# sash-a/CleanRL.jl

Measured on NVIDIA B200. Metric: ppo_env_steps_per_sec, higher is better.
Workload: dtype f32

## Files before the change

### cleanrl.jl_b200/csrc/rollout.cu

```cuda
#include "kernels.h"
#include "mlp_tile.cuh"

namespace {

constexpr int RE = 32;
constexpr int ROLL_FWD = CRL_THREADS;
constexpr int ROLL_THREADS = ROLL_FWD + 64;
constexpr int BIG_FWD = 128, BIG_THREADS = BIG_FWD + 64;
constexpr int BAR_FWD = 1, BAR_SPEC = 2, BAR_BOOK = 3;

__device__ __forceinline__ void nbar_sync(int id, int n) { asm volatile("bar.sync %0, %1;" ::"r"(id), "r"(n) : "memory"); }
__device__ __forceinline__ void nbar_arrive(int id, int n) { asm volatile("bar.arrive %0, %1;" ::"r"(id), "r"(n) : "memory"); }

template <int ENV> struct RolloutSmem {
  using G = TileGeom<4, 2>;
  using E = EnvTraits<ENV>;
  static constexpr int SP = G::S_PAD;
  static constexpr int PARAMS = 0;
  static constexpr int X = PARAMS + SmemParams<ENV>::SIZE;
  static constexpr int H1 = X + CRL_MAXD * SP;
  static constexpr int H2 = H1 + G::ROWS * SP;
  static constexpr int OUT = H2 + G::ROWS * SP;
  static constexpr int ST = OUT + 4 * RE;
  static constexpr int SPEC = ST + 4 * RE;
  static constexpr int RST = SPEC + 2 * 4 * RE;
  static constexpr int NOISE = RST + 4 * RE;
  static constexpr int USED = NOISE + 2 * RE;
  static constexpr int BOOK = USED + RE;
  static constexpr int FLOATS = BOOK + 4 * RE;
  static constexpr size_t BYTES = FLOATS * sizeof(float);
  static_assert((NOISE % 2) == 0, "the Float64 uniforms need 8-byte alignment");
};

#ifdef ROLL_TRACE
#define RTR(i) do { if (tr) tr[i] = clock64(); } while (0)
#else
#define RTR(i) do { } while (0)
#endif

template <int ENV> struct HeadRow { float w[CRL_H]; float b; };
template <int ENV> __device__ __forceinline__ void load_head_row(const float* sp, HeadRow<ENV>& hr) {
  using E = EnvTraits<ENV>;
  const int o = threadIdx.x / RE;
#pragma unroll
  for (int k = 0; k < CRL_H; k++) hr.w[k] = 0.0f;
  hr.b = 0.0f;
  if (threadIdx.x >= RE * (E::A + 1)) return;
  if (o < E::A) {
    const float* a = sp + SmemParams<ENV>::ACTOR;
#pragma unroll
    for (int k = 0; k < CRL_H; k++) hr.w[k] = a[NetOff<E::D, E::A>::W3 + k * E::A + o];
    hr.b = a[NetOff<E::D, E::A>::B3 + o];
  } else {
    const float* c = sp + SmemParams<ENV>::CRITIC;
#pragma unroll
    for (int k = 0; k < CRL_H; k++) hr.w[k] = c[NetOff<E::D, 1>::W3 + k];
    hr.b = c[NetOff<E::D, 1>::B3];
  }
}

template <int ENV, bool HEADREG = true, bool BOOKSYNC = false>
__device__ __forceinline__ void forward32(const ThreadCoord<TileGeom<4, 2>>& tc, float* smem, const HeadRow<ENV>& hr,
                                          long long* tr = nullptr) {
  using G = TileGeom<4, 2>;
  using E = EnvTraits<ENV>;
  using SM = RolloutSmem<ENV>;
  constexpr int SP = G::S_PAD;
  float* sp = smem + SM::PARAMS;
  float* xs = smem + SM::X;
  float* h1 = smem + SM::H1;
  float* h2 = smem + SM::H2;
  float* so = smem + SM::OUT;
  const float* np = sp + net_base<ENV>(tc.net);
  using NO = NetOff<E::D, 1>;
  RTR(0);
  tile_layer_fwd4<G, E::D>(tc, np + NO::W1, np + NO::B1, xs, h1 + tc.net * CRL_H * SP);
  RTR(1);
  nbar_sync(BAR_FWD, ROLL_FWD);
  RTR(2);
  tile_layer_fwd4<G, CRL_H>(tc, np + NO::W2, np + NO::B2, h1 + tc.net * CRL_H * SP, h2 + tc.net * CRL_H * SP);
  RTR(3);
  nbar_sync(BAR_FWD, ROLL_FWD);
  RTR(4);
  if (threadIdx.x < RE * (E::A + 1)) {
    const int o = threadIdx.x / RE, e = threadIdx.x % RE;
    const float* hrow = h2 + (o < E::A ? 0 : CRL_H) * SP + e;
    float hv[CRL_H];
#pragma unroll
    for (int k = 0; k < CRL_H; k++) hv[k] = hrow[k * SP];
    if (BOOKSYNC) nbar_sync(BAR_BOOK, RE * (E::A + 1) + 32);
    float acc = 0.0f;
    if (HEADREG) {
#pragma unroll
      for (int k = 0; k < CRL_H; k++) acc = fmaf(hr.w[k], hv[k], acc);
      acc += hr.b;
    } else if (o < E::A) {
      const float* a = sp + SmemParams<ENV>::ACTOR;
#pragma unroll
      for (int k = 0; k < CRL_H; k++) acc = fmaf(a[NetOff<E::D, E::A>::W3 + k * E::A + o], hv[k], acc);
      acc += a[NetOff<E::D, E::A>::B3 + o];
    } else {
      const float* c = sp + SmemParams<ENV>::CRITIC;
#pragma unroll
      for (int k = 0; k < CRL_H; k++) acc = fmaf(c[NetOff<E::D, 1>::W3 + k], hv[k], acc);
      acc += c[NetOff<E::D, 1>::B3];
    }
    so[o * RE + e] = acc;
  }
  RTR(5);
  nbar_sync(BAR_FWD, ROLL_FWD);
  RTR(6);
}

struct FwdCoord8x4 {
  int q, p, net, nb;
  __device__ FwdCoord8x4() {
    const int lane = threadIdx.x & 31, w = (threadIdx.x >> 5) & 3;
    q = w * 4 + (lane >> 3);
    p = lane & 7;
    net = q >> 3;
    nb = 8 * (q & 7);
  }
};
template <int K>
__device__ __forceinline__ void fwd_layer_8x4(const FwdCoord8x4& fc, const float* __restrict__ Wt, const float* __restrict__ bias,
                                              const float* __restrict__ in, float* __restrict__ out) {
  constexpr int SP = RE + 4, PF = 2;
  const float* wp = Wt + fc.nb;
  const float* ap = in + 4 * fc.p;
  const float4 b0 = *reinterpret_cast<const float4*>(bias + fc.nb), b1 = *reinterpret_cast<const float4*>(bias + fc.nb + 4);
  float2 acc[8][2];
#pragma unroll
  for (int j = 0; j < 8; j++) acc[j][0] = acc[j][1] = make_float2(0.0f, 0.0f);
  float4 w0[PF], w1[PF], av[PF];
#pragma unroll
  for (int i = 0; i < PF; i++) {
    if (i < K) {
      w0[i] = *reinterpret_cast<const float4*>(wp + i * CRL_H);
      w1[i] = *reinterpret_cast<const float4*>(wp + i * CRL_H + 4);
      av[i] = *reinterpret_cast<const float4*>(ap + i * SP);
    }
  }
#pragma unroll
  for (int k0 = 0; k0 < K; k0 += PF) {
    float4 w0n[PF], w1n[PF], avn[PF];
#pragma unroll
    for (int i = 0; i < PF; i++) {
      if (k0 + PF + i < K) {
        w0n[i] = *reinterpret_cast<const float4*>(wp + (k0 + PF + i) * CRL_H);
        w1n[i] = *reinterpret_cast<const float4*>(wp + (k0 + PF + i) * CRL_H + 4);
        avn[i] = *reinterpret_cast<const float4*>(ap + (k0 + PF + i) * SP);
      }
    }
#pragma unroll
    for (int i = 0; i < PF; i++) {
      if (k0 + i < K) {
        const float2 a01 = make_float2(av[i].x, av[i].y), a23 = make_float2(av[i].z, av[i].w);
#pragma unroll
        for (int j = 0; j < 8; j++) {
          const float wj = j < 4 ? f4_get(w0[i], j) : f4_get(w1[i], j - 4);
          const float2 ww = make_float2(wj, wj);
          acc[j][0] = __ffma2_rn(ww, a01, acc[j][0]);
          acc[j][1] = __ffma2_rn(ww, a23, acc[j][1]);
        }
      }
    }
#pragma unroll
    for (int i = 0; i < PF; i++) { w0[i] = w0n[i]; w1[i] = w1n[i]; av[i] = avn[i]; }
  }
#pragma unroll
  for (int j = 0; j < 8; j++) {
    const float b = j < 4 ? f4_get(b0, j) : f4_get(b1, j - 4);
    const float2 t0 = tanh_fast2(__fadd2_rn(acc[j][0], make_float2(b, b)));
    const float2 t1 = tanh_fast2(__fadd2_rn(acc[j][1], make_float2(b, b)));
    *reinterpret_cast<float4*>(out + (fc.nb + j) * SP + 4 * fc.p) = make_float4(t0.x, t0.y, t1.x, t1.y);
  }
}
template <int ENV, bool BOOKSYNC = false>
__device__ __forceinline__ void forward32_big(const FwdCoord8x4& fc, float* smem) {
  using E = EnvTraits<ENV>;
  using SM = RolloutSmem<ENV>;
  constexpr int SP = RE + 4;
  static_assert(SP == TileGeom<4, 2>::S_PAD, "both forward variants share one activation layout");
  float* sp = smem + SM::PARAMS;
  float* xs = smem + SM::X;
  float* h1 = smem + SM::H1;
  float* h2 = smem + SM::H2;
  float* so = smem + SM::OUT;
  const float* np = sp + net_base<ENV>(fc.net);
  using NO = NetOff<E::D, 1>;
  fwd_layer_8x4<E::D>(fc, np + NO::W1, np + NO::B1, xs, h1 + fc.net * CRL_H * SP);
  nbar_sync(BAR_FWD, BIG_FWD);
  fwd_layer_8x4<CRL_H>(fc, np + NO::W2, np + NO::B2, h1 + fc.net * CRL_H * SP, h2 + fc.net * CRL_H * SP);
  nbar_sync(BAR_FWD, BIG_FWD);
  if (threadIdx.x < RE * (E::A + 1)) {
    const int o = threadIdx.x / RE, e = threadIdx.x % RE;
    const float* hrow = h2 + (o < E::A ? 0 : CRL_H) * SP + e;
    if (BOOKSYNC) nbar_sync(BAR_BOOK, RE * (E::A + 1) + 32);
    float acc = 0.0f;
    if (o < E::A) {
      const float* a = sp + SmemParams<ENV>::ACTOR;
#pragma unroll 16
      for (int k = 0; k < CRL_H; k++) acc = fmaf(a[NetOff<E::D, E::A>::W3 + k * E::A + o], hrow[k * SP], acc);
      acc += a[NetOff<E::D, E::A>::B3 + o];
    } else {
      const float* c = sp + SmemParams<ENV>::CRITIC;
#pragma unroll 16
      for (int k = 0; k < CRL_H; k++) acc = fmaf(c[NetOff<E::D, 1>::W3 + k], hrow[k * SP], acc);
      acc += c[NetOff<E::D, 1>::B3];
    }
    so[o * RE + e] = acc;
  }
  nbar_sync(BAR_FWD, BIG_FWD);
}

template <int ENV, bool BIG>
__global__ void __launch_bounds__(BIG ? BIG_THREADS : ROLL_THREADS, BIG ? 2 : 1) rollout_kernel(RolloutArgs a) {
  constexpr int FWD = BIG ? BIG_FWD : ROLL_FWD;
  constexpr int SW0 = FWD / 32;
  using G = TileGeom<4, 2>;
  using E = EnvTraits<ENV>;
  using SM = RolloutSmem<ENV>;
  constexpr int SP = G::S_PAD;
  constexpr int D = E::D, A = E::A, S = E::S;
  constexpr bool CART = ENV == CRL_ENV_CARTPOLE;
  extern __shared__ __align__(16) float smem[];
  float* sp = smem + SM::PARAMS;
  float* xs = smem + SM::X;
  float* so = smem + SM::OUT;
  float* st_s = smem + SM::ST;
  float* spec_s = smem + SM::SPEC;
  float* rst_s = smem + SM::RST;
  double* noise_d = reinterpret_cast<double*>(smem + SM::NOISE);
  float* noise_f = smem + SM::NOISE;
  int* used_s = reinterpret_cast<int*>(smem + SM::USED);
  int* act_s = reinterpret_cast<int*>(smem + SM::BOOK);
  float* actf_s = smem + SM::BOOK + RE;
  float* rew_s = smem + SM::BOOK + 2 * RE;
  int* done_s = reinterpret_cast<int*>(smem + SM::BOOK + 3 * RE);
  const ThreadCoord<G> tc;
  const FwdCoord8x4 fc;

  load_params<ENV>(a.params, sp);
  for (int i = threadIdx.x; i < CRL_MAXD * SP; i += blockDim.x) xs[i] = 0.0f;

  const int warp = threadIdx.x >> 5;
  const int e = threadIdx.x & 31;
  const long long n = (long long)blockIdx.x * RE + e;
  const bool fwd = threadIdx.x < FWD;
  const bool owner = threadIdx.x < RE;
  const bool booker = warp == SW0 + 1;
  const bool in_range = n < a.N;
  const bool valid = owner && in_range;
  const unsigned long long step0 = a.ds->policy_step;
  const uint32_t gid = (uint32_t)(a.env_id_base + (int)n);

  float st[S];
  float obs[D];
  int env_t = 0;
  uint32_t resets = 0;
  bool done_flag = false;
  int ep_len = 0;
  double ep_ret = 0.0;
  bool prev_done = false;
  float obs_b[D];
  unsigned long long agg_n = 0;
  double agg_ret = 0.0, agg_len = 0.0, agg_max = -INFINITY;
  bool rec_pending = false;
  unsigned int rec_slot = 0;
  crl_episode rec;
  rec.step = 0; rec.env = 0; rec.length = 0; rec._pad = 0; rec.episode_return = 0.0;

#pragma unroll
  for (int i = 0; i < S; i++) st[i] = 0.0f;
#pragma unroll
  for (int k = 0; k < D; k++) obs_b[k] = 0.0f;
  if (valid) {
#pragma unroll
    for (int i = 0; i < S; i++) st[i] = a.env_state[n * S + i];
    env_t = a.env_t[n];
    resets = a.reset_count[n];
  }
  if (booker && in_range) {
    ep_len = a.ep_length[n];
    ep_ret = a.ep_return[n];
    resets = a.reset_count[n];
  }
  __syncthreads();
  HeadRow<ENV> hr;
  if (!BIG) load_head_row<ENV>(sp, hr);
  if (owner) {
    env_obs<ENV>(st, obs);
#pragma unroll
    for (int k = 0; k < D; k++) xs[k * SP + e] = obs[k];
#pragma unroll
    for (int i = 0; i < S; i++) st_s[i * RE + e] = st[i];
    used_s[e] = 0;
  }
  auto prepare_reset = [&]() {
    float u4[4], rs[S];
    int rt;
    rng_reset_uniforms(a.seed, gid, resets, u4);
    env_reset<ENV>(rs, rt, u4);
#pragma unroll
    for (int i = 0; i < S; i++) rst_s[i * RE + e] = rs[i];
  };
  if (booker && !a.reset_noise) prepare_reset();

  auto book = [&](int tb, const float (&zv)[A + 1], int act_i, float act_f, float r, bool dn) {
    const long long b = (long long)tb * a.N + n;
    ep_len += 1;
    float logprob;
    if (!E::CONT) {
      float m = zv[0];
#pragma unroll
      for (int k = 1; k < A; k++) m = fmaxf(m, zv[k]);
      float sum = 0.0f;
#pragma unroll
      for (int k = 0; k < A; k++) sum = __fadd_rn(sum, expf(__fsub_rn(zv[k], m)));
      const float ls = logf(sum);
      logprob = __fsub_rn(__fsub_rn(zv[0], m), ls);
#pragma unroll
      for (int k = 1; k < A; k++) logprob = (act_i == k) ? __fsub_rn(__fsub_rn(zv[k], m), ls) : logprob;
    } else {
      float lps = 0.0f;
#pragma unroll
      for (int k = 0; k < A; k++) {
        const float mean = zv[k];
        const float logstd = sp[SmemParams<ENV>::LOGSTD + k];
        const float sd = expf(logstd);
        const float diff = __fsub_rn(act_f, mean);
        const float q = __fdiv_rn(-__fmul_rn(diff, diff), __fmul_rn(__fmul_rn(2.0f, sd), sd));
        lps = __fadd_rn(lps, __fsub_rn(__fsub_rn(q, logstd), 0.9189385332046727f));
      }
      logprob = lps;
    }
    if (rec_pending) {
      if (rec_slot < (unsigned int)a.ep_capacity) a.records[rec_slot] = rec;
      rec_pending = false;
    }
    ep_ret += (double)r;
    if (in_range) {
      if (D == 4) {
        reinterpret_cast<float4*>(a.state)[b] = make_float4(obs_b[0], obs_b[1], obs_b[2], obs_b[3]);
      } else {
#pragma unroll
        for (int k = 0; k < D; k++) a.state[b * D + k] = obs_b[k];
      }
      if (!E::CONT) reinterpret_cast<int32_t*>(a.action)[b] = act_i;
      else reinterpret_cast<float*>(a.action)[b * A] = act_f;
      a.logprob[b] = logprob;
      a.value[b] = zv[A];
      a.terminal[b] = prev_done ? 1 : 0;
      a.reward[b] = r;
      if (dn) {
        rec_slot = atomicAdd(&a.eb->count, 1u);
        rec_pending = true;
        rec.step = tb; rec.env = (int)n; rec.length = ep_len; rec._pad = 0; rec.episode_return = ep_ret;
        agg_n += 1; agg_ret += ep_ret; agg_len += (double)ep_len; agg_max = fmax(agg_max, ep_ret);
        ep_ret = 0.0;
        ep_len = 0;
      }
    }
    prev_done = dn;
  };
  static_assert(!E::CONT || A == 1, "the Gaussian head hands one action per env to the bookkeeping warp");
  __syncthreads();

  for (int t = 0; t < a.T; t++) {
    if (!fwd) {
      if (booker) {
        float zv[A + 1];
#pragma unroll
        for (int k = 0; k <= A; k++) zv[k] = so[k * RE + e];
        const int act_i = act_s[e];
        const float act_f = actf_s[e], r = rew_s[e];
        const bool dn = done_s[e] != 0;
        nbar_arrive(BAR_BOOK, RE * (A + 1) + 32);
        if (t > 0) book(t - 1, zv, act_i, act_f, r, dn);
#pragma unroll
        for (int k = 0; k < D; k++) obs_b[k] = xs[k * SP + e];
        if (!a.reset_noise && used_s[e]) {
          resets += 1;
          prepare_reset();
          used_s[e] = 0;
        }
      }
      if (warp == SW0 && !a.action_noise) {
        if (!E::CONT) {
          noise_d[e] = in_range ? rng_action_uniform(a.seed, gid, step0 + (unsigned long long)t) : 0.0;
        } else {
          float zn[2] = {0.0f, 0.0f};
          if (in_range) rng_action_normals(a.seed, gid, step0 + (unsigned long long)t, zn);
          noise_f[e] = zn[0];
          noise_f[RE + e] = zn[1];
        }
      }
      if (CART) {
        float s4[4];
#pragma unroll
        for (int i = 0; i < 4; i++) s4[i] = st_s[i * RE + e];
        cartpole_dynamics(s4, warp - SW0);
#pragma unroll
        for (int i = 0; i < 4; i++) spec_s[((warp - SW0) * 4 + i) * RE + e] = s4[i];
      }
      __threadfence_block();
      nbar_arrive(BAR_SPEC, RE + 64);
    } else {
      if (BIG) forward32_big<ENV, true>(fc, smem); else forward32<ENV, true, true>(tc, smem, hr);
      if (owner) {
        const long long b = (long long)t * a.N + n;
        int act_i = 0;
        float act_f = 0.0f;
        if (!E::CONT) {
          float z[A], p[A];
#pragma unroll
          for (int k = 0; k < A; k++) z[k] = so[k * RE + e];
          float m = z[0];
#pragma unroll
          for (int k = 1; k < A; k++) m = fmaxf(m, z[k]);
          float ex[A], sum = 0.0f;
#pragma unroll
          for (int k = 0; k < A; k++) { ex[k] = expf(__fsub_rn(z[k], m)); sum = __fadd_rn(sum, ex[k]); }
          float psum = 0.0f;
#pragma unroll
          for (int k = 0; k < A; k++) {
            p[k] = __fdiv_rn(ex[k], sum);
            psum = __fadd_rn(psum, p[k]);
          }
          nbar_sync(BAR_SPEC, RE + 64);
          double u = 0.0;
          if (valid) u = a.action_noise ? a.action_noise[b] : noise_d[e];
          const double tt = __dmul_rn(u, (double)psum);
          float cw = p[0];
          int i = 0;
#pragma unroll
          for (int k = 1; k < A; k++) {
            if ((double)cw < tt && i == k - 1) { i = k; cw = __fadd_rn(cw, p[k]); }
          }
          act_i = i;
        } else {
          nbar_sync(BAR_SPEC, RE + 64);
          float zn = 0.0f;
          if (valid) zn = a.action_noise ? (float)a.action_noise[b * A] : noise_f[e];
          const float mean = so[e];
          const float sd = expf(sp[SmemParams<ENV>::LOGSTD]);
          act_f = __fadd_rn(mean, __fmul_rn(sd, zn));
        }
        float r;
        bool dn;
        if (CART) {
#pragma unroll
          for (int i = 0; i < 4; i++) st[i] = spec_s[(act_i * 4 + i) * RE + e];
          env_t += 1;
          cartpole_outcome(st, env_t, a.max_steps, r, dn);
        } else {
          pendulum_step(st, env_t, act_f, a.max_steps, r, dn);
        }
        env_obs<ENV>(st, obs);
        done_flag = dn;
        act_s[e] = act_i; actf_s[e] = act_f; rew_s[e] = r; done_s[e] = dn ? 1 : 0;
        if (valid && dn) {
          if (a.reset_noise) {
            const float4 v = reinterpret_cast<const float4*>(a.reset_noise)[b];
            const float u4[4] = {v.x, v.y, v.z, v.w};
            env_reset<ENV>(st, env_t, u4);
          } else {
#pragma unroll
            for (int i = 0; i < S; i++) st[i] = rst_s[i * RE + e];
            env_t = 0;
            used_s[e] = 1;
          }
          resets += 1;
          if (a.fresh_obs_after_reset) env_obs<ENV>(st, obs);
        }
#pragma unroll
        for (int k = 0; k < D; k++) xs[k * SP + e] = obs[k];
#pragma unroll
        for (int i = 0; i < S; i++) st_s[i * RE + e] = st[i];
      }
    }
    __syncthreads();
  }
  if (!fwd) {
    if (booker) {
      float zv[A + 1];
#pragma unroll
      for (int k = 0; k <= A; k++) zv[k] = so[k * RE + e];
      const int act_i = act_s[e];
      const float act_f = actf_s[e], r = rew_s[e];
      const bool dn = done_s[e] != 0;
      nbar_arrive(BAR_BOOK, RE * (A + 1) + 32);
      book(a.T - 1, zv, act_i, act_f, r, dn);
      if (rec_pending && rec_slot < (unsigned int)a.ep_capacity) a.records[rec_slot] = rec;
      if (in_range) {
        a.ep_length[n] = ep_len;
        a.ep_return[n] = ep_ret;
      }
      const double sr = warp_sum(agg_ret), sl = warp_sum(agg_len), mx = warp_max(agg_max);
      unsigned long long cn = agg_n;
#pragma unroll
      for (int o = 16; o > 0; o >>= 1) cn += __shfl_xor_sync(0xffffffffu, cn, o);
      if (e == 0 && cn > 0) {
        atomicAdd(&a.eb->n_episodes, cn);
        atomicAdd(&a.eb->sum_return, sr);
        atomicAdd(&a.eb->sum_length, sl);
        unsigned long long* addr = reinterpret_cast<unsigned long long*>(&a.eb->max_return);
        unsigned long long old = *addr, assumed;
        do {
          assumed = old;
          if (__longlong_as_double((long long)assumed) >= mx) break;
          old = atomicCAS(addr, assumed, (unsigned long long)__double_as_longlong(mx));
        } while (assumed != old);
      }
    }
    return;
  }

  float obs_last[D];
#pragma unroll
  for (int k = 0; k < D; k++) obs_last[k] = obs[k];
  if (owner) {
    float fresh[D];
    env_obs<ENV>(st, fresh);
#pragma unroll
    for (int k = 0; k < D; k++) xs[k * SP + e] = fresh[k];
  }
  nbar_sync(BAR_FWD, FWD);
  if (BIG) forward32_big<ENV, true>(fc, smem); else forward32<ENV, true, true>(tc, smem, hr);
  if (valid) {
    a.next_value[n] = so[A * RE + e];
#pragma unroll
    for (int i = 0; i < S; i++) a.env_state[n * S + i] = st[i];
    a.env_t[n] = env_t;
    a.reset_count[n] = resets;
#pragma unroll
    for (int k = 0; k < D; k++) a.next_obs[n * D + k] = obs_last[k];
    a.next_done[n] = done_flag ? 1 : 0;
  }
}

template <int ENV>
__global__ void env_step_raw_kernel(float* state, int* t, const void* action, float* reward, uint8_t* done,
                                    long long n, int max_steps) {
  constexpr int S = EnvTraits<ENV>::S;
  const long long i = (long long)blockIdx.x * blockDim.x + threadIdx.x;
  if (i >= n) return;
  float st[S];
#pragma unroll
  for (int k = 0; k < S; k++) st[k] = state[i * S + k];
  int tt = t[i];
  float r;
  bool dn;
  if (ENV == CRL_ENV_CARTPOLE) cartpole_step(st, tt, reinterpret_cast<const int32_t*>(action)[i], max_steps, r, dn);
  else pendulum_step(st, tt, reinterpret_cast<const float*>(action)[i], max_steps, r, dn);
#pragma unroll
  for (int k = 0; k < S; k++) state[i * S + k] = st[k];
  t[i] = tt;
  reward[i] = r;
  done[i] = dn ? 1 : 0;
}

template <int ENV>
__global__ void __launch_bounds__(CRL_THREADS) policy_forward_raw_kernel(const float* params, const float* obs,
                                                                         float* out_policy, float* logp,
                                                                         float* value, long long n) {
  using G = TileGeom<4, 2>;
  using E = EnvTraits<ENV>;
  using SM = RolloutSmem<ENV>;
  constexpr int SP = G::S_PAD;
  constexpr int D = E::D, A = E::A;
  extern __shared__ __align__(16) float smem[];
  float* xs = smem + SM::X;
  float* so = smem + SM::OUT;
  const ThreadCoord<G> tc;
  load_params<ENV>(params, smem + SM::PARAMS);
  const int e = threadIdx.x;
  const long long i = (long long)blockIdx.x * RE + e;
  if (e < RE) {
#pragma unroll
    for (int k = 0; k < D; k++) xs[k * SP + e] = i < n ? obs[i * D + k] : 0.0f;
  }
  __syncthreads();
  HeadRow<ENV> hr;
  load_head_row<ENV>(smem + SM::PARAMS, hr);
  forward32<ENV>(tc, smem, hr);
  if (e < RE && i < n) {
    float z[A];
#pragma unroll
    for (int k = 0; k < A; k++) { z[k] = so[k * RE + e]; out_policy[i * A + k] = z[k]; }
    value[i] = so[A * RE + e];
    if (!E::CONT) {
      float m = z[0];
#pragma unroll
      for (int k = 1; k < A; k++) m = fmaxf(m, z[k]);
      float sum = 0.0f;
#pragma unroll
      for (int k = 0; k < A; k++) sum = __fadd_rn(sum, expf(__fsub_rn(z[k], m)));
      const float ls = logf(sum);
#pragma unroll
      for (int k = 0; k < A; k++) logp[i * A + k] = __fsub_rn(__fsub_rn(z[k], m), ls);
    }
  }
}

template <int ENV> cudaError_t launch_rollout_t(const RolloutArgs& a, cudaStream_t s) {
  const int grid = (a.N + RE - 1) / RE;
  static int sms = 0;
  if (sms == 0) {
    int dev = 0;
    cudaGetDevice(&dev);
    cudaDeviceGetAttribute(&sms, cudaDevAttrMultiProcessorCount, dev);
  }
  if (grid > sms) rollout_kernel<ENV, true><<<grid, BIG_THREADS, RolloutSmem<ENV>::BYTES, s>>>(a);
  else rollout_kernel<ENV, false><<<grid, ROLL_THREADS, RolloutSmem<ENV>::BYTES, s>>>(a);
  return cudaGetLastError();
}

template <int ENV>
cudaError_t launch_policy_forward_t(const float* params, const float* obs, float* out_policy, float* logp,
                                    float* value, long long n, cudaStream_t s) {
  const long long grid = (n + RE - 1) / RE;
  if (grid == 0) return cudaSuccess;
  policy_forward_raw_kernel<ENV><<<(unsigned)grid, CRL_THREADS, RolloutSmem<ENV>::BYTES, s>>>(params, obs, out_policy,
                                                                                              logp, value, n);
  return cudaGetLastError();
}

__global__ void episode_buf_init_kernel(EpisodeBuf* eb) {
  eb->count = 0; eb->_pad = 0; eb->n_episodes = 0ull; eb->sum_return = 0.0; eb->sum_length = 0.0;
  eb->max_return = -INFINITY;
}

template <int ENV> cudaError_t init_attrs_t() {
  cudaError_t e = cudaFuncSetAttribute(rollout_kernel<ENV, false>, cudaFuncAttributeMaxDynamicSharedMemorySize,
                                       (int)RolloutSmem<ENV>::BYTES);
  if (e != cudaSuccess) return e;
  e = cudaFuncSetAttribute(rollout_kernel<ENV, true>, cudaFuncAttributeMaxDynamicSharedMemorySize, (int)RolloutSmem<ENV>::BYTES);
  if (e != cudaSuccess) return e;
  return cudaFuncSetAttribute(policy_forward_raw_kernel<ENV>, cudaFuncAttributeMaxDynamicSharedMemorySize,
                              (int)RolloutSmem<ENV>::BYTES);
}

}

cudaError_t kernels_init_rollout() {
  cudaError_t e = init_attrs_t<CRL_ENV_CARTPOLE>();
  if (e != cudaSuccess) return e;
  return init_attrs_t<CRL_ENV_PENDULUM>();
}

cudaError_t launch_episode_buf_init(EpisodeBuf* eb, cudaStream_t s) {
  episode_buf_init_kernel<<<1, 1, 0, s>>>(eb);
  return cudaGetLastError();
}

cudaError_t launch_rollout(int env_kind, const RolloutArgs& a, cudaStream_t s) {
  return env_kind == CRL_ENV_CARTPOLE ? launch_rollout_t<CRL_ENV_CARTPOLE>(a, s) : launch_rollout_t<CRL_ENV_PENDULUM>(a, s);
}

cudaError_t launch_env_step_raw(int env_kind, float* state, int* t, const void* action, float* reward,
                                uint8_t* done, long long n, int max_steps, cudaStream_t s) {
  if (n == 0) return cudaSuccess;
  const unsigned grid = (unsigned)((n + 127) / 128);
  if (env_kind == CRL_ENV_CARTPOLE)
    env_step_raw_kernel<CRL_ENV_CARTPOLE><<<grid, 128, 0, s>>>(state, t, action, reward, done, n, max_steps);
  else
    env_step_raw_kernel<CRL_ENV_PENDULUM><<<grid, 128, 0, s>>>(state, t, action, reward, done, n, max_steps);
  return cudaGetLastError();
}

cudaError_t launch_policy_forward_raw(int env_kind, const float* params, const float* obs, float* out_policy,
                                      float* logp, float* value, long long n, cudaStream_t s) {
  return env_kind == CRL_ENV_CARTPOLE
             ? launch_policy_forward_t<CRL_ENV_CARTPOLE>(params, obs, out_policy, logp, value, n, s)
             : launch_policy_forward_t<CRL_ENV_PENDULUM>(params, obs, out_policy, logp, value, n, s);
}

namespace {
template <int ENV>
__global__ void env_reset_kernel(int N, unsigned long long seed, int env_id_base, float* env_state, int* env_t,
                                 double* ep_return, int* ep_length, uint32_t* reset_count, float* next_obs,
                                 uint8_t* next_done) {
  constexpr int S = EnvTraits<ENV>::S, D = EnvTraits<ENV>::D;
  const int n = blockIdx.x * blockDim.x + threadIdx.x;
  if (n >= N) return;
  float u4[4], st[S], obs[D];
  const uint32_t k = reset_count[n];
  rng_reset_uniforms(seed, (uint32_t)(env_id_base + n), k, u4);
  int t;
  env_reset<ENV>(st, t, u4);
  env_obs<ENV>(st, obs);
#pragma unroll
  for (int i = 0; i < S; i++) env_state[n * S + i] = st[i];
#pragma unroll
  for (int i = 0; i < D; i++) next_obs[n * D + i] = obs[i];
  env_t[n] = t;
  reset_count[n] = k + 1;
  next_done[n] = 0;
  ep_return[n] = 0.0;
  ep_length[n] = 0;
}
template <int ENV>
__global__ void env_refresh_kernel(int N, const float* env_state, float* next_obs, uint8_t* next_done) {
  constexpr int S = EnvTraits<ENV>::S, D = EnvTraits<ENV>::D;
  const int n = blockIdx.x * blockDim.x + threadIdx.x;
  if (n >= N) return;
  float st[S], obs[D];
#pragma unroll
  for (int i = 0; i < S; i++) st[i] = env_state[n * S + i];
  env_obs<ENV>(st, obs);
#pragma unroll
  for (int i = 0; i < D; i++) next_obs[n * D + i] = obs[i];
  next_done[n] = 0;
}
}

cudaError_t launch_env_reset(int env_kind, int N, unsigned long long seed, int env_id_base, float* env_state,
                             int* env_t, double* ep_return, int* ep_length, uint32_t* reset_count, float* next_obs,
                             uint8_t* next_done, cudaStream_t s) {
  const int grid = (N + 127) / 128;
  if (env_kind == CRL_ENV_CARTPOLE)
    env_reset_kernel<CRL_ENV_CARTPOLE><<<grid, 128, 0, s>>>(N, seed, env_id_base, env_state, env_t, ep_return, ep_length,
                                                           reset_count, next_obs, next_done);
  else
    env_reset_kernel<CRL_ENV_PENDULUM><<<grid, 128, 0, s>>>(N, seed, env_id_base, env_state, env_t, ep_return, ep_length,
                                                           reset_count, next_obs, next_done);
  return cudaGetLastError();
}

cudaError_t launch_env_refresh(int env_kind, int N, const float* env_state, float* next_obs, uint8_t* next_done,
                               cudaStream_t s) {
  const int grid = (N + 127) / 128;
  if (env_kind == CRL_ENV_CARTPOLE) env_refresh_kernel<CRL_ENV_CARTPOLE><<<grid, 128, 0, s>>>(N, env_state, next_obs, next_done);
  else env_refresh_kernel<CRL_ENV_PENDULUM><<<grid, 128, 0, s>>>(N, env_state, next_obs, next_done);
  return cudaGetLastError();
}
```

Measured before the change: 249.9 million.

## Precompute first-layer activations for both CartPole action candidates speculatively

While the forward warps finish the current step, idle forward warps now compute layer-1 hidden activations for both speculative next CartPole states (one per discrete action). The next step's layer 1 is then a select between the two precomputed candidates, keyed on the chosen action stored in smem. This takes layer 1 off the serial critical path at the cost of doubling layer-1 work, adding another named barrier and using more shared memory. It only applies to the small-grid CartPole path without fresh observations after reset.

```diff
diff --git a/cleanrl.jl_b200/csrc/rollout.cu b/cleanrl.jl_b200/csrc/rollout.cu
--- a/cleanrl.jl_b200/csrc/rollout.cu
+++ b/cleanrl.jl_b200/csrc/rollout.cu
@@ -8,6 +8,8 @@
 constexpr int ROLL_THREADS = ROLL_FWD + 64;
 constexpr int BIG_FWD = 128, BIG_THREADS = BIG_FWD + 64;
 constexpr int BAR_FWD = 1, BAR_SPEC = 2, BAR_BOOK = 3;
+constexpr int BAR_CAND = 4;
+constexpr int CAND_THREADS = 192;
 
 __device__ __forceinline__ void nbar_sync(int id, int n) { asm volatile("bar.sync %0, %1;" ::"r"(id), "r"(n) : "memory"); }
 __device__ __forceinline__ void nbar_arrive(int id, int n) { asm volatile("bar.arrive %0, %1;" ::"r"(id), "r"(n) : "memory"); }
@@ -29,6 +31,9 @@
   static constexpr int BOOK = USED + RE;
   static constexpr int FLOATS = BOOK + 4 * RE;
   static constexpr size_t BYTES = FLOATS * sizeof(float);
+  static constexpr int XC = FLOATS;
+  static constexpr int HC = XC + 2 * CRL_MAXD * SP;
+  static constexpr size_t CAND_BYTES = (HC + 2 * G::ROWS * SP) * sizeof(float);
   static_assert((NOISE % 2) == 0, "the Float64 uniforms need 8-byte alignment");
 };
 
@@ -61,7 +66,7 @@
 
 template <int ENV, bool HEADREG = true, bool BOOKSYNC = false>
 __device__ __forceinline__ void forward32(const ThreadCoord<TileGeom<4, 2>>& tc, float* smem, const HeadRow<ENV>& hr,
-                                          long long* tr = nullptr) {
+                                          bool l1_cand = false, long long* tr = nullptr) {
   using G = TileGeom<4, 2>;
   using E = EnvTraits<ENV>;
   using SM = RolloutSmem<ENV>;
@@ -74,7 +79,20 @@
   const float* np = sp + net_base<ENV>(tc.net);
   using NO = NetOff<E::D, 1>;
   RTR(0);
-  tile_layer_fwd4<G, E::D>(tc, np + NO::W1, np + NO::B1, xs, h1 + tc.net * CRL_H * SP);
+  if (l1_cand) {
+    const float* hc = smem + SM::HC;
+    const int4 act = *reinterpret_cast<const int4*>(smem + SM::BOOK + tc.sb[0]);
+#pragma unroll
+    for (int j = 0; j < 4; j++) {
+      const int off = (tc.net * CRL_H + tc.jb[0] + j) * SP + tc.sb[0];
+      const float4 c0 = *reinterpret_cast<const float4*>(hc + off);
+      const float4 c1 = *reinterpret_cast<const float4*>(hc + G::ROWS * SP + off);
+      *reinterpret_cast<float4*>(h1 + off) =
+          make_float4(act.x ? c1.x : c0.x, act.y ? c1.y : c0.y, act.z ? c1.z : c0.z, act.w ? c1.w : c0.w);
+    }
+  } else {
+    tile_layer_fwd4<G, E::D>(tc, np + NO::W1, np + NO::B1, xs, h1 + tc.net * CRL_H * SP);
+  }
   RTR(1);
   nbar_sync(BAR_FWD, ROLL_FWD);
   RTR(2);
@@ -365,9 +383,12 @@
     prev_done = dn;
   };
   static_assert(!E::CONT || A == 1, "the Gaussian head hands one action per env to the bookkeeping warp");
+  const bool cand_on = !BIG && CART && !a.fresh_obs_after_reset;
+  const bool cand_warp = fwd && warp != 0 && warp != 4;
   __syncthreads();
 
   for (int t = 0; t < a.T; t++) {
+    const bool cand_step = cand_on && t + 1 < a.T;
     if (!fwd) {
       if (booker) {
         float zv[A + 1];
@@ -403,11 +424,32 @@
         cartpole_dynamics(s4, warp - SW0);
 #pragma unroll
         for (int i = 0; i < 4; i++) spec_s[((warp - SW0) * 4 + i) * RE + e] = s4[i];
+        if (cand_step) {
+          float* xc = smem + SM::XC + (warp - SW0) * CRL_MAXD * SP;
+#pragma unroll
+          for (int i = 0; i < 4; i++) xc[i * SP + e] = s4[i];
+        }
       }
       __threadfence_block();
       nbar_arrive(BAR_SPEC, RE + 64);
+      if (cand_step) nbar_arrive(BAR_CAND, 64 + CAND_THREADS);
     } else {
-      if (BIG) forward32_big<ENV, true>(fc, smem); else forward32<ENV, true, true>(tc, smem, hr);
+      if (BIG) forward32_big<ENV, true>(fc, smem); else forward32<ENV, true, true>(tc, smem, hr, cand_on && t > 0);
+      if (cand_step && cand_warp) {
+        nbar_sync(BAR_CAND, 64 + CAND_THREADS);
+        const int ci = (warp < 4 ? warp - 1 : warp - 2) * 32 + e;
+#pragma unroll 1
+        for (int u = ci; u < 2 * 2 * 16 * 8; u += CAND_THREADS) {
+          const int c = u >> 8, net = (u >> 7) & 1, q = (u >> 3) & 15, p = u & 7;
+          ThreadCoord<G> uc = tc;
+          uc.jb[0] = 4 * q;
+          uc.sb[0] = 4 * p;
+          const float* np = sp + net_base<ENV>(net);
+          using NO = NetOff<D, 1>;
+          tile_layer_fwd4<G, D>(uc, np + NO::W1, np + NO::B1, smem + SM::XC + c * CRL_MAXD * SP,
+                                smem + SM::HC + (c * G::ROWS + net * CRL_H) * SP);
+        }
+      }
       if (owner) {
         const long long b = (long long)t * a.N + n;
         int act_i = 0;
@@ -613,7 +655,7 @@
     cudaDeviceGetAttribute(&sms, cudaDevAttrMultiProcessorCount, dev);
   }
   if (grid > sms) rollout_kernel<ENV, true><<<grid, BIG_THREADS, RolloutSmem<ENV>::BYTES, s>>>(a);
-  else rollout_kernel<ENV, false><<<grid, ROLL_THREADS, RolloutSmem<ENV>::BYTES, s>>>(a);
+  else rollout_kernel<ENV, false><<<grid, ROLL_THREADS, RolloutSmem<ENV>::CAND_BYTES, s>>>(a);
   return cudaGetLastError();
 }
 
@@ -634,7 +676,7 @@
 
 template <int ENV> cudaError_t init_attrs_t() {
   cudaError_t e = cudaFuncSetAttribute(rollout_kernel<ENV, false>, cudaFuncAttributeMaxDynamicSharedMemorySize,
-                                       (int)RolloutSmem<ENV>::BYTES);
+                                       (int)RolloutSmem<ENV>::CAND_BYTES);
   if (e != cudaSuccess) return e;
   e = cudaFuncSetAttribute(rollout_kernel<ENV, true>, cudaFuncAttributeMaxDynamicSharedMemorySize, (int)RolloutSmem<ENV>::BYTES);
   if (e != cudaSuccess) return e;
```

Result: slower. 229.9 million, median of 6 (-8.0%).
